# resero-labs/latok

Hardware: AMD Instinct MI355X
Metric: input UTF-8 GB/s tokenized (fused feature+split-mask path) (higher is better)
Workload: dtype u64

## Files before the change

### latok_amd/csrc/split_kernels.hip

```cpp
#include <hip/hip_runtime.h>
#include <stdint.h>
#include <stdlib.h>

#include "bitscan.h"
#include "kernels.h"
#include "lane_math.h"
#include "utf8_decode.h"

namespace latok {

#ifdef LATOK_STAMPS
__device__ unsigned long long g_stamp_sum[16];
__device__ unsigned long long g_stamp_cnt;
#define LATOK_STAMP(k)                                                                           \
    do {                                                                                         \
        __builtin_amdgcn_sched_barrier(0);                                                       \
        unsigned long long t_;                                                                   \
        asm volatile("s_memtime %0\n\ts_waitcnt lgkmcnt(0)" : "=s"(t_)::"memory");            \
        __builtin_amdgcn_sched_barrier(0);                                                       \
        if ((k) > 0) stamp_acc[(k)] += t_ - stamp_prev;                                          \
        stamp_prev = t_;                                                                         \
    } while (0)
#else
#define LATOK_STAMP(k) do { } while (0)
// ... 1124 lines not shown
__device__ __attribute__((noinline, cold)) void tables_fetch_bytes(const uint8_t* t1, const uint8_t* t2, uint8_t* tables, int* ctl) {
    const int lane = (int)(threadIdx.x & 63u);
    struct { const uint8_t* t1; const uint8_t* t2; } P = {t1, t2};
    struct { uint8_t* tables; int* ctl; } L = {tables, ctl};
    typedef const void __attribute__((address_space(1))) * gptr_t;
    typedef void __attribute__((address_space(3))) * lptr_t;
    for (;;) {
        const int ticket = __hip_atomic_fetch_add(&L.ctl[0], 1, __ATOMIC_RELAXED, __HIP_MEMORY_SCOPE_WORKGROUP);
        const int g = __builtin_amdgcn_readfirstlane(ticket) >> 6;
        if (g >= kLazyGrabs) break;
        if (g == kLazyGrabs - 1) {
#pragma unroll
            for (int j = 0; j < 4; ++j) {
                const lk_lead_entry e = lk_lead_entry_of((uint32_t)(64 * j + lane));
                reinterpret_cast<uint2*>(L.tables + kLdsLeadTab)[64 * j + lane] = make_uint2(e.sel, e.hi0);
            }
        } else {
#pragma unroll
            for (int j = 0; j < kLazyPer; ++j) {
                const int row = g * kLazyPer + j;
                if (row < kLazyRows)
                    __builtin_amdgcn_global_load_lds((gptr_t)(P.t1 + 1024 * row + 16 * lane), (lptr_t)(L.tables + 1024 * row), 16, 0, 0);
            }
            __builtin_amdgcn_s_waitcnt(0x0F70);
        }
        __hip_atomic_fetch_add(&L.ctl[1], 1, __ATOMIC_RELEASE, __HIP_MEMORY_SCOPE_WORKGROUP);
    }
    while (__hip_atomic_load(&L.ctl[1], __ATOMIC_ACQUIRE, __HIP_MEMORY_SCOPE_WORKGROUP) < 64 * kLazyGrabs) __builtin_amdgcn_s_sleep(2);
}

template <int MODE = kModeBits>
__device__ __forceinline__ TileLds wave_lds(uint8_t* lds, int wave) {
    TileLds L;
    L.t1 = lds;
    L.t2 = lds + kStage1Pad;
    uint8_t* const w = lds + lds_shift(MODE);
    uint8_t* mine = wave < kWPB ? w + kLdsWaves + wave * kWaveLdsBytes : lds + lds_total(MODE) + (wave - kWPB) * kWaveLdsBytes;
    L.stage = mine;
    L.halo = mine + kStageBytes;
    L.bw = reinterpret_cast<lk_u64*>(mine + kStageBytes + 16);
    L.lut = lds;
    L.ltab = lds + kLdsLeadTab;
    L.tables = lds;
    L.ctl = reinterpret_cast<int*>(w + kLdsMisc) + 16;
    L.t1b = lds;
    L.t2b = lds + kB6Stage1Bytes;
    L.ctab = mode_base(MODE) == kModeBytes ? lds + kLdsByteCodes : L.lut + kSliceLutBytes;
    L.small_bits = L.small_space = nullptr;
    return L;
}

#ifdef LATOK_STAMPS
#define LATOK_STAMP_ARG , stamp_acc
#define LATOK_STAMP_PARAM , unsigned long long* stamp_acc
#define LATOK_STAMP_NULL , nullptr
#else
#define LATOK_STAMP_ARG
#define LATOK_STAMP_PARAM
#define LATOK_STAMP_NULL
#endif

template <int MODE, bool FAST_TAIL = false, int WPB = kWPB, int PF = kCpsPrefetchRows>
__device__ __forceinline__ void run_segment(const SplitParams& P, uint8_t* lds, int64_t seg, int tid, int lane,
                                            int wave, bool tables LATOK_STAMP_PARAM) {
    const int S = P.seg_tiles;
    const TileLds L = wave_lds<MODE>(lds, wave);
    int4* sm = reinterpret_cast<int4*>(lds + lds_shift(MODE) + kLdsSumm);
    ScanLdsT<WPB>& scan = *reinterpret_cast<ScanLdsT<WPB>*>(lds + lds_shift(MODE) + kLdsScan);

    const int64_t T0 = seg * S;
    const int64_t T1 = min(T0 + S, P.n_tiles);
    const int n_seg = (int)(T1 - T0);
    int64_t tfv = 0;
    if (wave + WPB * lane < n_seg) tfv = P.tile_first[T0 + wave + WPB * lane];
    tfv = tfv < 0 ? 0 : (tfv > P.n_str ? P.n_str : tfv);
    if (tables) __syncthreads();
    constexpr bool kDefer = mode_writes_bits(MODE) && !mode_is_bytes(MODE);
    lk_u64 obuf[8];
    int slot = 0, k_first = wave;
    const int64_t n_words = (P.total + 63) >> 6;
    auto flush = [&]() {
#pragma unroll
        for (int j = 0; j < 8; ++j) {
            if (j < slot) {
                const int64_t w = (T0 + k_first + j * WPB) * 64 + lane;
                if (w < n_words) P.bits_out[w] = obuf[j];
            }
        }
        slot = 0;
    };
    auto put = [&](lk_u64 w, int k) {
        if (slot == 0) k_first = k;
#pragma unroll
        for (int j = 0; j < 8; ++j) obuf[j] = (j == slot) ? w : obuf[j];
        if (++slot == 8) flush();
    };
    CpsPrefetch pf;
    pf.valid = false;
    for (int k = wave, j = 0; k < n_seg; k += WPB, ++j) {
        const lk_u64 w = process_tile<MODE, kDefer, false, FAST_TAIL, PF>(P, L, T0 + k, lane_read64(tfv, j), 0, -1, true, &sm[k], lane LATOK_STAMP_ARG
                                                                      , MODE == kModeBits && !FAST_TAIL ? &pf : nullptr, k + WPB < n_seg ? T0 + k + WPB : (int64_t)-1
                                                                      );
        if (kDefer) put(w, k);
#ifdef LATOK_STAMPS
        stamp_acc[0] += 1;
#endif
    }
    if (kDefer) flush();
    __syncthreads();
    {
        Fn64 f = fn_identity();
        Hd64 h = hd_identity();
        if (tid < n_seg) {
            const int4 s = sm[tid];
            P.summ[T0 + tid] = s;
            f = fn_of(s);
            h.h = s.z; h.c = s.w & 1;
        }
        Fn64 ef, tfn; Hd64 eh, th;
        block_scan<WPB>(f, h, scan, &ef, &eh, &tfn, &th);
        if (tid == 0) { P.seg_fn[seg] = tfn; P.seg_hd[seg] = th; }
    }
    __syncthreads();
}

template <int MODE, bool FAST_TAIL = false, int PF = kCpsPrefetchRows>
__global__ __launch_bounds__(tile_wpb(MODE) * 64) void k_tiles_main(SplitParams P) {
    constexpr int WPB = tile_wpb(MODE);
    __shared__ __attribute__((aligned(16))) uint8_t lds[lds_total_tiles(MODE)];
    const int tid = threadIdx.x;
    const int lane = tid & 63;
    const int wave = __builtin_amdgcn_readfirstlane(tid >> 6);
    if (blockIdx.x == 0 && tid == 0) *P.fix_count = 0;

    bool tables = MODE != kModeBlockMask;
    if (tables) {
        if (mode_base(MODE) == kModeBytes) load_tables_ascii_bytes(lds, P);
        else load_tables<WPB * 64, MODE>(lds, P);
    }
#ifdef LATOK_STAMPS
    unsigned long long stamp_acc[16];
    for (int i = 0; i < 16; ++i) stamp_acc[i] = 0;
#endif
    for (int64_t seg = blockIdx.x; seg < P.n_segs; seg += gridDim.x) {
        run_segment<MODE, FAST_TAIL, WPB, PF>(P, lds, seg, tid, lane, wave, tables LATOK_STAMP_ARG);
        tables = false;
    }
#ifdef LATOK_STAMPS
    if (lane == 0)
        for (int i = 0; i < 16; ++i) atomicAdd(&g_stamp_sum[i], stamp_acc[i]);
#endif
}

template <int MODE, int NW, bool ONE>
__device__ __forceinline__ void resolve_segments(const SplitParams& P, uint8_t* lds, int tid, int lane, int wave) {
    const int S = P.seg_tiles;
    ScanLdsT<NW>& scan = *reinterpret_cast<ScanLdsT<NW>*>(lds + lds_shift(MODE) + kLdsScan);
    int* misc = reinterpret_cast<int*>(lds + lds_shift(MODE) + kLdsMisc);
    int* fix_t = reinterpret_cast<int*>(lds + lds_shift(MODE) + kLdsTf);
    int2* fix_in = reinterpret_cast<int2*>(lds + lds_shift(MODE) + kLdsSumm);
    bool tables_loaded = ONE;

    for (int64_t seg = ONE ? 0 : (int64_t)blockIdx.x; seg < (ONE ? 1 : P.n_segs); seg += ONE ? 1 : (int64_t)gridDim.x) {
        const int64_t T0 = seg * S;
        const int64_t T1 = min(T0 + S, P.n_tiles);
        const int n_seg = (int)(T1 - T0);
        if (tid == 0) misc[0] = 0;
        const int64_t t = T0 + tid;
        int4 s = make_int4(0, 0, 0, 0);
        if (tid < n_seg) s = P.summ[t];
        Fn64 pf = fn_identity();
        Hd64 sh = hd_identity();
        if (P.n_segs > 1) {
            const int64_t per = (P.n_segs + NW * 64 - 1) / (NW * 64);
            const int64_t lo = min((int64_t)tid * per, P.n_segs), hi = min(lo + per, P.n_segs);
            Fn64 f = fn_identity();
            Hd64 h = hd_identity();
            for (int64_t j = lo; j < hi; ++j) {
                if (j < seg) f = fn_then(f, P.seg_fn[j]);
                if (j > seg) h = hd_then(h, P.seg_hd[j]);
            }
            Fn64 ef; Hd64 eh;
            block_scan<NW>(f, h, scan, &ef, &eh, &pf, &sh);
        }
        const long long q_seg_in = fn_apply(pf, 0);
        Hd64 rest; rest.h = sh.h; rest.c = 1;

        Fn64 f = fn_identity();
        Hd64 h = hd_identity();
        if (tid < n_seg) {
            f = fn_of(s);
            h.h = s.z; h.c = s.w & 1;
        }
        Fn64 ef, tfn; Hd64 eh, th;
        block_scan<NW>(f, h, scan, &ef, &eh, &tfn, &th);
        if (tid < n_seg) {
            const long long q_in = fn_apply(ef, q_seg_in);
            const long long q_end = fn_apply(f, q_in);
            const long long h_next = hd_then(eh, rest).h;
            const int tz = (q_end + h_next) > 0;
            const int tz0 = s.y > 0;
            if (q_in != 0 || tz != tz0) {
                const int geom = s.w;
                if (!mode_rules(MODE) && (MODE == kModeBits || mode_is_bytes(MODE)) && (geom & 1) && q_in <= 1 &&
                    (q_in == 0 || s.z == 0)) {
                    const int64_t t0 = t * kTile;
                    const int64_t t_end = min(t0 + kTile, P.total);
                    auto lead_back = [&](int64_t lo, int64_t hi) -> int {
                        int back = 0;
                        if (mode_base(MODE) == kModeBytes && ((geom >> 30) & 1)) {
                            if (hi > t_end) hi = t_end;
                            while (back < 3 && hi - 1 - back > lo && (P.u8[hi - 1 - back] & 0xC0u) == 0x80u) ++back;
                        }
                        return back;
                    };
                    if (q_in == 1) {
                        const int64_t hi = t0 + ((geom >> 1) & 0x1FFF);
                        const int keep = (geom >> 27) & 1;
                        clear_range(P.bits_out, t0, hi, t_end, 0, keep, keep ? lead_back(t0, hi) : 0);
                    }
                    if (tz != tz0) {
                        const int64_t lo = t0 + ((geom >> 14) & 0x1FFF);
                        const int keep = (geom >> 29) & 1;
                        clear_range(P.bits_out, lo, t_end, t_end, (geom >> 28) & 1, keep, keep ? lead_back(lo, t_end) : 0);
                    }
                } else {
                    const int slot = atomicAdd(&misc[0], 1);
                    fix_t[slot] = tid;
                    fix_in[slot] = make_int2((int)(q_in < (1 << 20) ? q_in : (1 << 20)), tz);
                }
            }
        }
        __syncthreads();
        const int n_fix = misc[0];
        if (n_fix > 0) {
            if (!tables_loaded && MODE != kModeBlockMask) {
                load_tables<NW * 64, MODE>(lds, P);
                tables_loaded = true;
                __syncthreads();
            }
            const TileLds L = wave_lds<MODE>(lds, wave);
            for (int i = wave; i < n_fix; i += NW) {
                const int64_t tt = T0 + fix_t[i];
                const int2 in = fix_in[i];
                const int64_t idx0 = wave_lower_bound(P.row_off, P.n_str + 1, tt * kTile, lane);
                process_tile<MODE>(P, L, tt, idx0, in.x, in.y, false, nullptr, lane);
            }
            if (tid == 0) atomicAdd(reinterpret_cast<unsigned long long*>(P.fix_count), (unsigned long long)n_fix);
        }
        __syncthreads();
    }
}

template <int MODE, int NW>
__global__ __launch_bounds__(NW * 64) void k_resolve_fix(SplitParams P) {
    __shared__ __attribute__((aligned(16))) uint8_t lds[lds_total(MODE)];
    const int tid = threadIdx.x;
    const int lane = tid & 63;
    const int wave = __builtin_amdgcn_readfirstlane(tid >> 6);
    resolve_segments<MODE, NW, false>(P, lds, tid, lane, wave);
    signal_block_done(P.done);
}

__device__ __forceinline__ void tile_index_entry(const int64_t* __restrict__ row_off, int64_t n_str, int64_t n_tiles,
                                                 int64_t* __restrict__ tile_first, int64_t s, int lane) {
    int64_t w0 = 0, w1 = -1;
    if (s <= n_str) {
        const int64_t p = row_off[s];
        const int64_t prev = s > 0 ? row_off[s - 1] : -1;
        w0 = prev < 0 ? 0 : prev / kTile + 1;
        w1 = p / kTile;
        if (w1 > n_tiles - 1) w1 = n_tiles - 1;
    }
    const bool wide = w1 - w0 >= 16;
    if (!wide)
        for (int64_t w = w0; w <= w1; ++w) tile_first[w] = s;
    unsigned long long m = __ballot(wide);
    while (m) {
        const int src = __ffsll((long long)m) - 1;
        m &= m - 1;
        const int64_t a = lane_read64(w0, src), b = lane_read64(w1, src), v = lane_read64(s, src);
        for (int64_t w = a + lane; w <= b; w += 64) tile_first[w] = v;
    }
}


template <int MODE>
__global__ __launch_bounds__(kWPB * 64) void k_one_segment(SplitParams P) {
    __shared__ __attribute__((aligned(16))) uint8_t lds[lds_total(MODE)];
    const int tid = threadIdx.x;
    const int lane = tid & 63;
    const int wave = __builtin_amdgcn_readfirstlane(tid >> 6);
    if (tid == 0) *P.fix_count = 0;
    load_tables<kWPB * 64, MODE>(lds, P);
    for (int64_t base = 0; base <= P.n_str; base += kWPB * 64)
        tile_index_entry(P.row_off, P.n_str, P.n_tiles, P.tile_first, base + tid, lane);
    __threadfence_block();
    __syncthreads();
    run_segment<MODE, true>(P, lds, 0, tid, lane, wave, true LATOK_STAMP_NULL);
    __threadfence_block();
    __syncthreads();
    resolve_segments<MODE, kWPB, true>(P, lds, tid, lane, wave);
    signal_block_done(P.done);
}

__global__ void k_any_nonzero(const int8_t* __restrict__ a1, const int8_t* __restrict__ a2, int64_t n,
                              int* __restrict__ flags) {
    int f1 = 0, f2 = 0;
    for (int64_t i = (int64_t)blockIdx.x * blockDim.x + threadIdx.x; i < n; i += (int64_t)gridDim.x * blockDim.x) {
        f1 |= a1[i] != 0;
        f2 |= a2[i] != 0;
    }
    if (__any(f1) && (threadIdx.x & 63) == 0) atomicOr(&flags[0], 1);
    if (__any(f2) && (threadIdx.x & 63) == 0) atomicOr(&flags[1], 1);
}

hipError_t launch_any_nonzero(const int8_t* a1, const int8_t* a2, int64_t n, int* flags, hipStream_t st) {
    hipError_t e = hipMemsetAsync(flags, 0, 2 * sizeof(int), st);
    if (e != hipSuccess || n <= 0) return e;
    int64_t blocks = (n + 255) / 256;
    if (blocks > 1024) blocks = 1024;
    hipLaunchKernelGGL(k_any_nonzero, dim3((unsigned)blocks), dim3(256), 0, st, a1, a2, n, flags);
    return hipGetLastError();
}

__device__ __forceinline__ uint32_t swar_add_u8(uint32_t a, uint32_t b) {
    return ((a & 0x7F7F7F7Fu) + (b & 0x7F7F7F7Fu)) ^ ((a ^ b) & 0x80808080u);
}
struct FeatSums {
    uint32_t v[7];
};
__device__ __forceinline__ FeatSums feat_popc(const lk_planes& F, lk_u64 m) {
    FeatSums r;
#pragma unroll
    for (int j = 0; j < 7; ++j) r.v[j] = 0;
#pragma unroll
    for (int c = 0; c < LK_N_FEATURES; ++c)
        r.v[c >> 2] |= (uint32_t)__popcll(LK_PLANE_GET(F, c) & m) << (8 * (c & 3));
    return r;
}
template <int HI>
__device__ __forceinline__ FeatSums feat_popc_half(const lk_planes& F, uint32_t m) {
    FeatSums r;
#pragma unroll
    for (int j = 0; j < 7; ++j) r.v[j] = 0;
#pragma unroll
    for (int c = 0; c < LK_N_FEATURES; ++c)
        r.v[c >> 2] |= (uint32_t)__popc(LK_PLANE_HALF(F, c, HI) & m) << (8 * (c & 3));
    return r;
}
__device__ __forceinline__ uint32_t feat_row_bits1(uint32_t w, uint32_t p, uint32_t x, uint32_t y, bool first, bool last) {
    uint32_t r = w & 0xFFFu;
    r |= ((p >> 0) & 1u) << 12; r |= ((x >> 0) & 1u) << 13; r |= ((p >> 1) & 1u) << 14; r |= ((x >> 1) & 1u) << 15;
    r |= ((p >> 3) & 1u) << 16; r |= ((x >> 3) & 1u) << 17;
    r |= (first ? 1u : (p >> 5) & 1u) << 18; r |= (last ? 1u : (x >> 5) & 1u) << 19;
    r |= ((p >> 6) & 1u) << 20; r |= ((x >> 8) & 1u) << 21; r |= ((x >> 10) & 1u) << 22;
    r |= ((y >> 0) & 1u) << 23; r |= ((y >> 10) & 1u) << 24;
    return r;
}

constexpr int kFeatWaves = 7;
constexpr int kFeatRound = 896;
constexpr int kFeatRec = 25;
constexpr int kFeatRoundTm = 768;
constexpr int kFeatWinBytes = kFeatRound * kFeatRec + 16;
static_assert(kFeatRoundTm * (kFeatRec + 2) + 16 <= kFeatWinBytes, "token-major round fits the window");
constexpr int kFeatWaveLds = kFeatWinBytes + 16 + 66 * 8;
constexpr int kFeatLdsTotal = kFeatWaves * kFeatWaveLds;
static_assert(kFeatLdsTotal <= 160 * 1024, "LDS budget of one CU");
static_assert(kFeatWinBytes % 16 == 0 && kFeatWaveLds % 16 == 0, "alignment");

__device__ __forceinline__ void put_record(uint8_t* win, int slot, const FeatSums& s) {
    uint8_t* rec = win + slot * kFeatRec;
#pragma unroll
    for (int q = 0; q < 6; ++q) __builtin_memcpy(rec + 4 * q, &s.v[q], 4);
    rec[24] = (uint8_t)s.v[6];
}
__device__ __forceinline__ int record_shift(const void* dst) { return (int)((uintptr_t)dst & 15u); }
__device__ __forceinline__ void flush_records(const uint8_t* win, int n_rec, uint8_t* dst, int lane) {
    const int n_bytes = n_rec * 25;
    const uint8_t* src = win + record_shift(dst);
    const int head = min((16 - record_shift(dst)) & 15, n_bytes);
    if (lane < head) dst[lane] = src[lane];
    const int n_vec = (n_bytes - head) >> 4;
    for (int i = lane; i < n_vec; i += 64) {
        const u32x4 v = *reinterpret_cast<const u32x4*>(src + head + 16 * i);
        __builtin_nontemporal_store(v, reinterpret_cast<u32x4*>(dst + head + 16 * i));
    }
    const int tail0 = head + 16 * n_vec;
    if (lane < n_bytes - tail0) dst[tail0 + lane] = src[tail0 + lane];
}
template <typename OUT>
constexpr int span_round() { return kFeatWinBytes / (4 * (int)sizeof(OUT)) < kFeatRound ? kFeatWinBytes / (4 * (int)sizeof(OUT)) : kFeatRound; }

__device__ __forceinline__ void load_codes64(const uint8_t* __restrict__ p, uint32_t (&d)[16]) {
    const u32x4* q = reinterpret_cast<const u32x4*>(p);
#pragma unroll
    for (int k = 0; k < 4; ++k) {
        const u32x4 v = q[k];
        d[4 * k + 0] = v.x; d[4 * k + 1] = v.y; d[4 * k + 2] = v.z; d[4 * k + 3] = v.w;
    }
}

template <typename OUT>
__device__ __forceinline__ void feature_tile(const FeatParams& P, const TileLds& L, int64_t t, int lane) {
    OUT* const spans4 = reinterpret_cast<OUT*>(P.spans4);
    const int64_t t0 = t * kTile;
    const int64_t total = P.total;
    const int64_t n_words = (total + 63) >> 6;
    const int64_t w = t * 64 + lane;
    const int n_wave = (int)P.tile_cnt[t];
    if (n_wave == 0) return;
    const lk_u64 x = w < n_words ? P.kept[w] : 0ull;
    const int off = w < n_words ? (int)P.word_pref[w] : 0;
    const int64_t base_out = P.tile_rank[t];
    const lk_u64 xb = w < n_words ? P.bits[w] : 0ull;

    int64_t idx0 = P.tile_first[t];
    idx0 = idx0 < 0 ? 0 : (idx0 > P.n_str ? P.n_str : idx0);
    const int64_t start_before = idx0 > 0 ? P.row_off[idx0 - 1] : 0;
    int64_t ro = idx0 + lane <= P.n_str ? P.row_off[idx0 + lane] : INT64_MAX;
    const int64_t base = t0 + 64 * (int64_t)lane;
    const int64_t remain = total - base;
    const lk_u64 valid = remain >= 64 ? ~0ull : (remain <= 0 ? 0ull : ((1ull << remain) - 1ull));
    uint32_t d[16];
    load_codes64(P.codes + base, d);
    uint32_t edge = 0;
    if (lane == 0 && t0 > 0) edge = P.codes[t0 - 1];
    if (lane == 63) {
        if (t0 + kTile < total) edge = P.codes[t0 + kTile];
        if (t0 + kTile + 1 < total) edge |= (uint32_t)P.codes[t0 + kTile + 1] << 8;
    }
    L.bw[lane] = 0;
    if (lane < 2) L.bw[64 + lane] = 0;
    wave_lds_sync();
    for (;;) {
// ... 486 lines not shown
        s_lo[lane] = (int)lo_in;
        wave_lds_sync();
        OUT* spans4 = reinterpret_cast<OUT*>(S.items);
        for (int k0 = 0; k0 < n_items; k0 += 64) {
            const int k = k0 + lane;
            FeatSums sum;
#pragma unroll
            for (int j = 0; j < 7; ++j) sum.v[j] = 0;
            if (k < n_items) {
                int wl = 0, wh = 64;
                while (wh - wl > 1) {
                    const int mid = (wl + wh) >> 1;
                    if (s_pref[mid] <= k) wl = mid; else wh = mid;
                }
                lk_u64 m = s_items[wl];
                for (int r = k - s_pref[wl]; r > 0; --r) m &= m - 1ull;
                const int b = lk_ctz(m);
                const int64_t a = 64 * (int64_t)wl + b;
                const int64_t e = next_set_bit(s_bits, a + 1, total);
                const int64_t a2 = next_zero_bit(s_space, a, e);
                const int64_t e2 = prev_zero_end(s_space, a2, e);
                const lk_u64 bl = L.bw[wl] & ((2ull << b) - 1ull);
                const int64_t lo = bl ? 64 * (int64_t)wl + 63 - __builtin_clzll(bl) : (int64_t)s_lo[wl];
                OUT* rec = spans4 + 4 * (int64_t)k;
                rec[0] = (OUT)(a - lo); rec[1] = (OUT)(e - lo); rec[2] = (OUT)(a2 - lo); rec[3] = (OUT)(e2 - lo);
                uint32_t acc[LK_N_FEATURES];
#pragma unroll
                for (int c = 0; c < LK_N_FEATURES; ++c) acc[c] = 0;
                for (int64_t w = wl; 64 * w < e; ++w) {
                    lk_u64 msk = ~0ull;
                    if (w == wl) msk &= ~0ull << b;
                    if (e < 64 * w + 64) msk &= (1ull << (e - 64 * w)) - 1ull;
#pragma unroll
                    for (int c = 0; c < LK_N_FEATURES; ++c) acc[c] += (uint32_t)__popcll(s_planes[w * LK_N_FEATURES + c] & msk);
                }
#pragma unroll
                for (int c = 0; c < LK_N_FEATURES; ++c) sum.v[c >> 2] |= (acc[c] & 0xFFu) << (8 * (c & 3));
            }
            const int n_here = min(64, n_items - k0);
            uint8_t* const fdst = reinterpret_cast<uint8_t*>(S.features) + (int64_t)k0 * kFeatRec;
            if (k < n_items) put_record(s_win + record_shift(fdst), lane, sum);
            wave_lds_sync();
            flush_records(s_win, n_here, fdst, lane);
            wave_lds_sync();
        }
    }
    OUT* out = reinterpret_cast<OUT*>(S.items);
    lk_u64 rest = KIND == 2 ? 0ull : x;
    int k = inc - cnt;
    while (rest) {
        const int b = lk_ctz(rest);
        rest &= rest - 1;
        const lk_u64 bl = Bw & ((2ull << b) - 1ull);
        const int64_t lo = bl ? base + 63 - __builtin_clzll(bl) : lo_in;
        if (KIND == 0) {
            out[k] = (OUT)(base + b - lo);
        } else {
            const lk_u64 above = xb & (~1ull << b);
            int64_t a2, e2;
            if (above) {
                const int eb = lk_ctz(above);
                const lk_u64 seg = nn & (~0ull << b) & ((1ull << eb) - 1ull);
                a2 = base + lk_ctz(seg);
                e2 = base + 64 - __builtin_clzll(seg);
            } else if (xb1) {
                const int eb = lk_ctz(xb1);
                const lk_u64 seg0 = nn & (~0ull << b);
                const lk_u64 seg1 = nn1 & ((1ull << eb) - 1ull);
                a2 = seg0 ? base + lk_ctz(seg0) : base + 64 + lk_ctz(seg1);
                e2 = seg1 ? base + 128 - __builtin_clzll(seg1) : base + 64 - __builtin_clzll(seg0);
            } else {
                const int64_t e = next_set_bit(s_bits, base + 64, total);
                const lk_u64 seg = nn & (~0ull << b);
                a2 = seg ? base + lk_ctz(seg) : next_zero_bit(s_space, base + 64, e);
                e2 = prev_zero_end(s_space, a2, e);
            }
            out[2 * k] = (OUT)(a2 - lo);
            out[2 * k + 1] = (OUT)(e2 - lo);
        }
        ++k;
    }
    if (S.done) {
        __threadfence_system();
        if (lane == 0) __hip_atomic_store(S.done, S.seq, __ATOMIC_RELAXED, __HIP_MEMORY_SCOPE_SYSTEM);
    }
}

hipError_t launch_small_batch(const SplitParams& P, bool rules, int kind, bool out32, void* counts, void* items, int8_t* features,
                              int64_t* n_items, unsigned long long* done, unsigned long long seq, hipStream_t st) {
    SmallParams S;
    S.P = P;
    S.counts = counts;
    S.items = items;
    S.features = features;
    S.n_items = n_items;
    S.done = done;
    S.seq = seq;
#define LATOK_SB(M, K, T) hipLaunchKernelGGL((k_small_batch<M, K, T>), dim3(1), dim3(64), 0, st, S)
#define LATOK_SB_K(M, T) do { if (kind == 0) LATOK_SB(M, 0, T); else if (kind == 1) LATOK_SB(M, 1, T); else LATOK_SB(M, 2, T); } while (0)
    if (rules) {
        if (out32) LATOK_SB_K(kModeRules, int32_t); else LATOK_SB_K(kModeRules, int64_t);
    } else {
        if (out32) LATOK_SB_K(kModeBits, int32_t); else LATOK_SB_K(kModeBits, int64_t);
    }
#undef LATOK_SB_K
#undef LATOK_SB
    return hipGetLastError();
}

__global__ __launch_bounds__(64) void k_small_block_mask(SmallParams S) {
    __shared__ __attribute__((aligned(16))) uint8_t lds[kWaveLdsBytes];
    __shared__ int s_flags[2];
    const int lane = threadIdx.x;
    TileLds L;
    L.t1 = L.t2 = L.lut = L.ctab = L.ltab = L.t1b = L.t2b = nullptr; L.tables = nullptr; L.ctl = nullptr;
    L.small_bits = L.small_space = nullptr;
    L.stage = lds;
    L.halo = lds + kStageBytes;
    L.bw = reinterpret_cast<lk_u64*>(lds + kStageBytes + 16);
    SplitParams P = S.P;
    const int64_t n = P.total;
    uint32_t f1 = 0, f2 = 0;
    for (int64_t i = 4 * (int64_t)lane; i < n; i += 256) {
        if (i + 4 <= n) {
            f1 |= *reinterpret_cast<const uint32_t*>(P.bm_a1 + i);
            f2 |= *reinterpret_cast<const uint32_t*>(P.bm_a2 + i);
        } else {
            for (int64_t j = i; j < n; ++j) { f1 |= (uint8_t)P.bm_a1[j]; f2 |= (uint8_t)P.bm_a2[j]; }
        }
    }
    const int any1 = __any(f1 != 0u), any2 = __any(f2 != 0u);
    if (lane == 0) { s_flags[0] = any1; s_flags[1] = any2; }
    wave_lds_sync();
    P.bm_flags = s_flags;
    process_tile<kModeBlockMask, false, true, true>(P, L, 0, 0, 0, -1, false, nullptr, lane);
    if (S.done) {
        __threadfence_system();
        if (lane == 0) __hip_atomic_store(S.done, S.seq, __ATOMIC_RELAXED, __HIP_MEMORY_SCOPE_SYSTEM);
    }
}

hipError_t launch_small_block_mask(const SplitParams& P, unsigned long long* done, unsigned long long seq, hipStream_t st) {
    SmallParams S;
    S.P = P;
    S.counts = S.items = nullptr;
    S.features = nullptr;
    S.n_items = nullptr;
    S.done = done;
    S.seq = seq;
    hipLaunchKernelGGL(k_small_block_mask, dim3(1), dim3(64), 0, st, S);
    return hipGetLastError();
}

__global__ __launch_bounds__(256) void k_tile_index(const int64_t* __restrict__ row_off, int64_t n_str, int64_t n_tiles,
                                                   int64_t* __restrict__ tile_first) {
    tile_index_entry(row_off, n_str, n_tiles, tile_first, (int64_t)blockIdx.x * blockDim.x + threadIdx.x, threadIdx.x & 63);
}

hipError_t launch_tile_index(const SplitParams& P, hipStream_t st) {
    if (P.n_tiles <= 0) return hipSuccess;
    const int64_t entries = P.n_str + 1;
    hipLaunchKernelGGL(k_tile_index, dim3((unsigned)((entries + 255) / 256)), dim3(256), 0, st, P.row_off, P.n_str, P.n_tiles,
                       P.tile_first);
    return hipGetLastError();
}

void plan_segments(int64_t n_tiles, int n_cu, int* seg_tiles, int64_t* n_segs) {
    const int64_t per_cu = (n_tiles + n_cu - 1) / n_cu;
    const int64_t rounds = per_cu > kSegMax ? (per_cu + kSegMax - 1) / kSegMax : 1;
    int64_t s = (n_tiles + (int64_t)n_cu * rounds - 1) / ((int64_t)n_cu * rounds);
    if (s < kWPB) s = kWPB;
    if (s > kSegMax) s = kSegMax;
    *seg_tiles = (int)s;
    *n_segs = (n_tiles + s - 1) / s;
}

void plan_launch(int64_t n_tiles, int n_cu, bool in_flow, int mode, bool one_launch_ok, LaunchPlan* L) {
    const int wpb = tile_wpb(mode);
    int n_cu_eff = n_cu;
    if (in_flow && n_cu >= 64) {
        const int cand[3] = {n_cu * 7 / 8, n_cu * 13 / 16, n_cu * 3 / 4};
        int best = cand[0], best_fill = -1;
        for (int c = 0; c < 3; ++c) {
            int st_ = 0;
            int64_t ns_ = 0;
            plan_segments(n_tiles, cand[c], &st_, &ns_);
            const int fill = (st_ - 1) % wpb + 1;
            if (fill * 2 >= wpb) { best = cand[c]; break; }
            if (fill > best_fill) { best = cand[c]; best_fill = fill; }
        }
        n_cu_eff = best;
    }
    if (n_cu_eff < 8) n_cu_eff = n_cu < 8 ? n_cu : 8;
    L->n_cu_eff = n_cu_eff;
    plan_segments(n_tiles, n_cu_eff, &L->seg_tiles, &L->n_segs);
    L->one_launch = one_launch_ok && n_tiles <= kOneSegTiles && (mode == kModeBits || mode == kModeRules);
    if (L->one_launch) {
        L->seg_tiles = (int)(n_tiles < kOneSegTiles ? kOneSegTiles : n_tiles);
        L->n_segs = 1;
    }
    L->grid = L->one_launch ? 1 : (int)(L->n_segs < n_cu ? (L->n_segs < 1 ? 1 : L->n_segs) : n_cu);
    L->rounds = (L->n_segs + L->grid - 1) / L->grid;
    L->fast_tail = !L->one_launch && n_tiles <= kFastTailTiles && (mode == kModeBits || mode == kModeRules);
    L->pf = mode == kModeBits && in_flow && !L->fast_tail && !L->one_launch ? kCpsPrefetchRowsFlow : kCpsPrefetchRows;
    L->wpb = L->one_launch ? kWPB : wpb;
    const bool narrow_resolve = mode == kModeBits || mode == kModeBytes || mode == kModeLatin1 || mode == kModeUcs2;
    L->nw = L->one_launch || !narrow_resolve ? kWPB : (L->seg_tiles <= 128 ? 2 : (L->seg_tiles <= 256 ? 4 : kWPB));
}

hipError_t launch_split_tiles(const SplitParams& P, int mode, const LaunchPlan& L, hipStream_t st) {
    const dim3 grid(L.grid), block(kWPB * 64);
    if (mode == kModeBits && L.pf == kCpsPrefetchRowsFlow) hipLaunchKernelGGL((k_tiles_main<kModeBits, false, kCpsPrefetchRowsFlow>), grid, block, 0, st, P);
    else if (mode == kModeBits && L.fast_tail) hipLaunchKernelGGL((k_tiles_main<kModeBits, true>), grid, block, 0, st, P);
    else if (mode == kModeRules && L.fast_tail) hipLaunchKernelGGL((k_tiles_main<kModeRules, true>), grid, block, 0, st, P);
    else if (mode == kModeBits) hipLaunchKernelGGL((k_tiles_main<kModeBits>), grid, block, 0, st, P);
    else if (mode == kModeValues) hipLaunchKernelGGL((k_tiles_main<kModeValues>), grid, block, 0, st, P);
    else if (mode == kModeRules) hipLaunchKernelGGL((k_tiles_main<kModeRules>), grid, block, 0, st, P);
    else if (mode == kModeBytes) hipLaunchKernelGGL((k_tiles_main<kModeBytes>), grid, dim3(tile_wpb(kModeBytes) * 64), 0, st, P);
    else if (mode == kModeLatin1) hipLaunchKernelGGL((k_tiles_main<kModeLatin1>), grid, dim3(tile_wpb(kModeLatin1) * 64), 0, st, P);
    else if (mode == kModeUcs2) hipLaunchKernelGGL((k_tiles_main<kModeUcs2>), grid, dim3(tile_wpb(kModeUcs2) * 64), 0, st, P);
    else if (mode == kModeBytesRules) hipLaunchKernelGGL((k_tiles_main<kModeBytesRules>), grid, block, 0, st, P);
    else if (mode == kModeLatin1Rules) hipLaunchKernelGGL((k_tiles_main<kModeLatin1Rules>), grid, block, 0, st, P);
    else if (mode == kModeUcs2Rules) hipLaunchKernelGGL((k_tiles_main<kModeUcs2Rules>), grid, block, 0, st, P);
    else if (mode == kModeValuesRules) hipLaunchKernelGGL((k_tiles_main<kModeValuesRules>), grid, block, 0, st, P);
    else hipLaunchKernelGGL((k_tiles_main<kModeBlockMask>), grid, block, 0, st, P);
    return hipGetLastError();
}

hipError_t launch_one_segment(const SplitParams& P, int mode, hipStream_t st) {
    if (P.n_segs != 1 || P.seg_tiles < P.n_tiles || P.n_tiles > kOneSegTiles || (mode != kModeBits && mode != kModeRules))
        return hipErrorInvalidValue;
    if (mode == kModeBits) hipLaunchKernelGGL((k_one_segment<kModeBits>), dim3(1), dim3(kWPB * 64), 0, st, P);
    else hipLaunchKernelGGL((k_one_segment<kModeRules>), dim3(1), dim3(kWPB * 64), 0, st, P);
    return hipGetLastError();
}

hipError_t launch_resolve_fix(const SplitParams& P, int mode, const LaunchPlan& L, hipStream_t st) {
    if (L.nw * 64 < P.seg_tiles) return hipErrorInvalidValue;
    const dim3 grid(L.grid), block(kWPB * 64);
#define LATOK_RESOLVE_NW(M)                                                                            \
    if (L.nw == 2) hipLaunchKernelGGL((k_resolve_fix<M, 2>), grid, dim3(128), 0, st, P);               \
    else if (L.nw == 4) hipLaunchKernelGGL((k_resolve_fix<M, 4>), grid, dim3(256), 0, st, P);          \
    else hipLaunchKernelGGL((k_resolve_fix<M, kWPB>), grid, block, 0, st, P)
    if (mode == kModeBits) { LATOK_RESOLVE_NW(kModeBits); }
    else if (mode == kModeValues) hipLaunchKernelGGL((k_resolve_fix<kModeValues, kWPB>), grid, block, 0, st, P);
    else if (mode == kModeRules) hipLaunchKernelGGL((k_resolve_fix<kModeRules, kWPB>), grid, block, 0, st, P);
    else if (mode == kModeBytesRules) hipLaunchKernelGGL((k_resolve_fix<kModeBytesRules, kWPB>), grid, block, 0, st, P);
    else if (mode == kModeLatin1Rules) hipLaunchKernelGGL((k_resolve_fix<kModeLatin1Rules, kWPB>), grid, block, 0, st, P);
    else if (mode == kModeUcs2Rules) hipLaunchKernelGGL((k_resolve_fix<kModeUcs2Rules, kWPB>), grid, block, 0, st, P);
    else if (mode == kModeValuesRules) hipLaunchKernelGGL((k_resolve_fix<kModeValuesRules, kWPB>), grid, block, 0, st, P);
    else if (mode == kModeBytes) { LATOK_RESOLVE_NW(kModeBytes); }
    else if (mode == kModeLatin1) { LATOK_RESOLVE_NW(kModeLatin1); }
    else if (mode == kModeUcs2) { LATOK_RESOLVE_NW(kModeUcs2); }
    else hipLaunchKernelGGL((k_resolve_fix<kModeBlockMask, kWPB>), grid, block, 0, st, P);
#undef LATOK_RESOLVE_NW
    return hipGetLastError();
}

#ifdef LATOK_STAMPS
extern "C" int latok_diag_stamps(unsigned long long* out16, int reset) {
    hipError_t e = hipMemcpyFromSymbol(out16, HIP_SYMBOL(g_stamp_sum), 16 * sizeof(unsigned long long));
    if (reset) {
        unsigned long long z[16] = {0};
        (void)hipMemcpyToSymbol(HIP_SYMBOL(g_stamp_sum), z, sizeof(z));
    }
    return (int)e;
}
#endif

}
```

Baseline: 1505.

## Add slim resolve kernel for bits mode and vectorize tile index build

Adds a k_resolve_slim kernel for bits mode. It uses a compact LDS layout with no table load, and moves the rare fix-up recompute into a noinline cold function that reloads params from the kernarg segment. This cuts LDS and register pressure so more workgroups fit per CU (waves_per_eu hints, with a static_assert for 7 groups per CU). Separately, k_tile_index now has each thread handle several pairs of row offsets with 16-byte vector loads, which reduces grid size and redundant loads. The risk is that fewer waves handle the fix-ups and that the cold call adds overhead when fix-ups are frequent.

```diff
diff --git a/latok_amd/csrc/split_kernels.hip b/latok_amd/csrc/split_kernels.hip
--- a/latok_amd/csrc/split_kernels.hip
+++ b/latok_amd/csrc/split_kernels.hip
@@ -1300,13 +1300,49 @@
 #endif
 }
 
-template <int MODE, int NW, bool ONE>
+constexpr int kSlimLdsScan = 0;
+constexpr int kSlimLdsMisc = 512;
+constexpr int kSlimLdsFix = kSlimLdsMisc + 256;
+constexpr int slim_lds_fix_in(int nw) { return kSlimLdsFix + nw * 64 * 4; }
+constexpr int slim_lds_waves(int nw) { return slim_lds_fix_in(nw) + nw * 64 * 8; }
+constexpr int slim_fix_waves(int nw) { return nw == 4 ? 3 : nw; }
+constexpr int slim_lds_total(int nw) { return slim_lds_waves(nw) + slim_fix_waves(nw) * kWaveLdsBytes; }
+static_assert(7 * slim_lds_total(4) <= 160 * 1024, "7 workgroups of k_resolve_slim<4> per CU");
+static_assert(slim_lds_waves(2) % 16 == 0 && kWaveLdsBytes % 16 == 0, "alignment");
+__device__ __forceinline__ SplitParams kernarg_split_params() {
+    typedef const void __attribute__((address_space(4))) * kernarg_t;
+    SplitParams P;
+    __builtin_memcpy(&P, (kernarg_t)__builtin_amdgcn_kernarg_segment_ptr(), sizeof(P));
+    return P;
+}
+template <int NW>
+__device__ __attribute__((noinline, cold)) void resolve_recompute_slim(uint8_t* wave_buf, const int* fix_t, const int2* fix_in,
+                                                                       int n_fix, int64_t T0, int wave) {
+    const SplitParams P = kernarg_split_params();
+    const int lane = (int)(threadIdx.x & 63u);
+    TileLds L;
+    L.t1 = P.t1;
+    L.t2 = P.t2;
+    L.lut = L.ctab = L.ltab = L.t1b = L.t2b = nullptr; L.tables = nullptr; L.ctl = nullptr;
+    L.stage = wave_buf;
+    L.halo = wave_buf + kStageBytes;
+    L.bw = reinterpret_cast<lk_u64*>(wave_buf + kStageBytes + 16);
+    L.small_bits = L.small_space = nullptr;
+    for (int i = wave; i < n_fix; i += slim_fix_waves(NW)) {
+        const int64_t tt = T0 + fix_t[i];
+        const int2 in = fix_in[i];
+        const int64_t idx0 = wave_lower_bound(P.row_off, P.n_str + 1, tt * kTile, lane);
+        process_tile<kModeBits>(P, L, tt, idx0, in.x, in.y, false, nullptr, lane);
+    }
+}
+
+template <int MODE, int NW, bool ONE, bool SLIM = false>
 __device__ __forceinline__ void resolve_segments(const SplitParams& P, uint8_t* lds, int tid, int lane, int wave) {
     const int S = P.seg_tiles;
-    ScanLdsT<NW>& scan = *reinterpret_cast<ScanLdsT<NW>*>(lds + lds_shift(MODE) + kLdsScan);
-    int* misc = reinterpret_cast<int*>(lds + lds_shift(MODE) + kLdsMisc);
-    int* fix_t = reinterpret_cast<int*>(lds + lds_shift(MODE) + kLdsTf);
-    int2* fix_in = reinterpret_cast<int2*>(lds + lds_shift(MODE) + kLdsSumm);
+    ScanLdsT<NW>& scan = *reinterpret_cast<ScanLdsT<NW>*>(lds + (SLIM ? kSlimLdsScan : lds_shift(MODE) + kLdsScan));
+    int* misc = reinterpret_cast<int*>(lds + (SLIM ? kSlimLdsMisc : lds_shift(MODE) + kLdsMisc));
+    int* fix_t = reinterpret_cast<int*>(lds + (SLIM ? kSlimLdsFix : lds_shift(MODE) + kLdsTf));
+    int2* fix_in = reinterpret_cast<int2*>(lds + (SLIM ? slim_lds_fix_in(NW) : lds_shift(MODE) + kLdsSumm));
     bool tables_loaded = ONE;
 
     for (int64_t seg = ONE ? 0 : (int64_t)blockIdx.x; seg < (ONE ? 1 : P.n_segs); seg += ONE ? 1 : (int64_t)gridDim.x) {
@@ -1381,7 +1417,13 @@
         }
         __syncthreads();
         const int n_fix = misc[0];
-        if (n_fix > 0) {
+        if constexpr (SLIM) {
+            if (n_fix > 0) {
+                if (wave < n_fix && wave < slim_fix_waves(NW))
+                    resolve_recompute_slim<NW>(lds + slim_lds_waves(NW) + wave * kWaveLdsBytes, fix_t, fix_in, n_fix, T0, wave);
+                if (tid == 0) atomicAdd(reinterpret_cast<unsigned long long*>(P.fix_count), (unsigned long long)n_fix);
+            }
+        } else if (n_fix > 0) {
             if (!tables_loaded && MODE != kModeBlockMask) {
                 load_tables<NW * 64, MODE>(lds, P);
                 tables_loaded = true;
@@ -1410,12 +1452,20 @@
     signal_block_done(P.done);
 }
 
-__device__ __forceinline__ void tile_index_entry(const int64_t* __restrict__ row_off, int64_t n_str, int64_t n_tiles,
-                                                 int64_t* __restrict__ tile_first, int64_t s, int lane) {
+template <int NW>
+__global__ __launch_bounds__(NW * 64) __attribute__((amdgpu_waves_per_eu(NW == 4 ? 7 : 5, 8))) void k_resolve_slim(SplitParams P) {
+    __shared__ __attribute__((aligned(16))) uint8_t lds[slim_lds_total(NW)];
+    const int tid = threadIdx.x;
+    const int lane = tid & 63;
+    const int wave = __builtin_amdgcn_readfirstlane(tid >> 6);
+    resolve_segments<kModeBits, NW, false, true>(P, lds, tid, lane, wave);
+    signal_block_done(P.done);
+}
+
+__device__ __forceinline__ void tile_index_entry_of(int64_t p, int64_t prev, int64_t n_str, int64_t n_tiles,
+                                                    int64_t* __restrict__ tile_first, int64_t s, int lane) {
     int64_t w0 = 0, w1 = -1;
     if (s <= n_str) {
-        const int64_t p = row_off[s];
-        const int64_t prev = s > 0 ? row_off[s - 1] : -1;
         w0 = prev < 0 ? 0 : prev / kTile + 1;
         w1 = p / kTile;
         if (w1 > n_tiles - 1) w1 = n_tiles - 1;
@@ -1430,6 +1480,15 @@
         const int64_t a = lane_read64(w0, src), b = lane_read64(w1, src), v = lane_read64(s, src);
         for (int64_t w = a + lane; w <= b; w += 64) tile_first[w] = v;
     }
+}
+__device__ __forceinline__ void tile_index_entry(const int64_t* __restrict__ row_off, int64_t n_str, int64_t n_tiles,
+                                                 int64_t* __restrict__ tile_first, int64_t s, int lane) {
+    int64_t p = 0, prev = -1;
+    if (s <= n_str) {
+        p = row_off[s];
+        if (s > 0) prev = row_off[s - 1];
+    }
+    tile_index_entry_of(p, prev, n_str, n_tiles, tile_first, s, lane);
 }
 
 
@@ -2222,16 +2281,42 @@
     return hipGetLastError();
 }
 
+constexpr int kIndexPairs = 4;
+constexpr int kIndexPerBlock = 256 * 2 * kIndexPairs;
 __global__ __launch_bounds__(256) void k_tile_index(const int64_t* __restrict__ row_off, int64_t n_str, int64_t n_tiles,
                                                    int64_t* __restrict__ tile_first) {
-    tile_index_entry(row_off, n_str, n_tiles, tile_first, (int64_t)blockIdx.x * blockDim.x + threadIdx.x, threadIdx.x & 63);
+    const int lane = threadIdx.x & 63;
+    const int64_t e0 = ((int64_t)blockIdx.x * 4 + (threadIdx.x >> 6)) * (128 * kIndexPairs) + 2 * lane;
+    const bool vec = (reinterpret_cast<uintptr_t>(row_off) & 15) == 0;
+    int64_t a[kIndexPairs], b[kIndexPairs], pv[kIndexPairs];
+#pragma unroll
+    for (int j = 0; j < kIndexPairs; ++j) {
+        const int64_t e = e0 + 128 * j;
+        a[j] = b[j] = 0;
+        pv[j] = -1;
+        if (vec && e + 1 <= n_str) {
+            const longlong2 v = *reinterpret_cast<const longlong2*>(row_off + e);
+            a[j] = v.x;
+            b[j] = v.y;
+        } else {
+            if (e <= n_str) a[j] = row_off[e];
+            if (e + 1 <= n_str) b[j] = row_off[e + 1];
+        }
+        if (e > 0 && e <= n_str) pv[j] = row_off[e - 1];
+    }
+#pragma unroll
+    for (int j = 0; j < kIndexPairs; ++j) {
+        const int64_t e = e0 + 128 * j;
+        tile_index_entry_of(a[j], pv[j], n_str, n_tiles, tile_first, e, lane);
+        tile_index_entry_of(b[j], a[j], n_str, n_tiles, tile_first, e + 1, lane);
+    }
 }
 
 hipError_t launch_tile_index(const SplitParams& P, hipStream_t st) {
     if (P.n_tiles <= 0) return hipSuccess;
     const int64_t entries = P.n_str + 1;
-    hipLaunchKernelGGL(k_tile_index, dim3((unsigned)((entries + 255) / 256)), dim3(256), 0, st, P.row_off, P.n_str, P.n_tiles,
-                       P.tile_first);
+    hipLaunchKernelGGL(k_tile_index, dim3((unsigned)((entries + kIndexPerBlock - 1) / kIndexPerBlock)), dim3(256), 0, st, P.row_off,
+                       P.n_str, P.n_tiles, P.tile_first);
     return hipGetLastError();
 }
 
@@ -2312,7 +2397,11 @@
     if (L.nw == 2) hipLaunchKernelGGL((k_resolve_fix<M, 2>), grid, dim3(128), 0, st, P);               \
     else if (L.nw == 4) hipLaunchKernelGGL((k_resolve_fix<M, 4>), grid, dim3(256), 0, st, P);          \
     else hipLaunchKernelGGL((k_resolve_fix<M, kWPB>), grid, block, 0, st, P)
-    if (mode == kModeBits) { LATOK_RESOLVE_NW(kModeBits); }
+    if (mode == kModeBits) {
+        if (L.nw == 2) hipLaunchKernelGGL((k_resolve_slim<2>), grid, dim3(128), 0, st, P);
+        else if (L.nw == 4) hipLaunchKernelGGL((k_resolve_slim<4>), grid, dim3(256), 0, st, P);
+        else hipLaunchKernelGGL((k_resolve_slim<kWPB>), grid, block, 0, st, P);
+    }
     else if (mode == kModeValues) hipLaunchKernelGGL((k_resolve_fix<kModeValues, kWPB>), grid, block, 0, st, P);
     else if (mode == kModeRules) hipLaunchKernelGGL((k_resolve_fix<kModeRules, kWPB>), grid, block, 0, st, P);
     else if (mode == kModeBytesRules) hipLaunchKernelGGL((k_resolve_fix<kModeBytesRules, kWPB>), grid, block, 0, st, P);
```

Result: slower. 1483 (-1.4%).
